# rofuyu/exp-trmf-nips16

Hardware: AMD Instinct MI355X
Metric: als_iterations_per_sec (higher is better)
Workload: dtype f32

## Files before the change

### exp-trmf-nips16_amd/csrc/session.hpp

```cpp
#pragma once

#include "session_xphase.hpp"

extern "C" char **environ;

namespace trmf {

struct TrmfSessionImpl : SessionXPhase {
    ~TrmfSessionImpl() {
        if (stream) (void)hipStreamSynchronize(stream);
        if (side) (void)hipStreamSynchronize(side);
        if (aux_theta) (void)hipStreamSynchronize(aux_theta);
        for (auto &e : events) {
            hipEvent_t all[] = {e.f0, e.fk0, e.fk1, e.f1, e.xg1, e.x1, e.lv1};
            for (hipEvent_t ev : all) if (ev) (void)hipEventDestroy(ev);
        }
        for (hipEvent_t ev : {gx0, gx1, gx2, fs0, fs1, fs2, ts0, ts1}) if (ev) (void)hipEventDestroy(ev);
        release_p2p();
        for (hipEvent_t ev : {ov_b, ov_c[0], ov_c[1], ov_c[2], ov_c[3], emu_ready, emu_end}) if (ev) (void)hipEventDestroy(ev);
        if (side) (void)hipStreamDestroy(side);
        for (hipEvent_t ev : {theta_fork, theta_done}) if (ev) (void)hipEventDestroy(ev);
        if (cg_note) (void)hipHostFree(cg_note);
        StreamCache::release(aux_theta);
        StreamCache::release(stream);
// ... 73 lines not shown
        for (double x : h) acc += x;
        *out = acc;
        return 0;
    }
    int device_sum_squares(const real *dv, size_t count, double *out) { return launch_sum_squares(dv, count) || finish_sum_squares(out) ? kFail : 0; }
    size_t footprint_estimate() const {
        const size_t sz = sizeof(real), NVb = (size_t)(T + 1) * KP * sz, NHb = (size_t)(n + 1) * KP * sz;
        size_t b = dense ? 2 * (size_t)T * n * sz + (full ? (size_t)kGemmChunks * std::max(T, n) * KP * sz : 0)
                         : 2 * (size_t)nnz * (4 + sz) + ((size_t)T + n + 2) * 4;
        b += NVb + NHb + (size_t)(T + n) * k * sz;
        b += 11 * NVb + 4 * NVb;
        if (!full) b += (size_t)T * k * k * sz;
        if (full) b += NHb;
        if (generic) b += (size_t)std::min(kGenBlocks, std::max(n, 1)) * k * k * sz;
        b += (size_t)kLogCap * sizeof(DeviceIterLog) + ((size_t)32 << 20);
        return b + b / 16;
    }
    int create(const PyMatrix *Y, const uint32_t *lags, uint32_t lag_size, const PyMatrix *Wm,
               const PyMatrix *Hm, const PyMatrix *LVm) {
        T = (int)Y->rows; n = (int)Y->cols; k = (int)Wm->cols; nnz = Y->nnz;
        KP = padded_rank(k); NT = KP / kTile; KMAX = ((k + 7) / 8) * 8;
        generic = k > kMaxRank;
        nlag = (int)lag_size; midx = nlag ? (int)lags[nlag - 1] : 0;
        comm = active_comm();
        if (StreamCache::acquire(&stream)) return kFail;
        FillStreamScope fill(stream);
        dense = Y->type != TRMF_SPARSE;
        DevicePool::current().reserve(footprint_estimate());

        const double tu0 = now_s();
        if (!dense) {
            host_row_ptr.assign(Y->row_ptr, Y->row_ptr + (size_t)T + 1);
            host_col_ptr.assign(Y->col_ptr, Y->col_ptr + (size_t)n + 1);
            if (upload_ptr32(Yc_ptr, Y->col_ptr, (size_t)n + 1)) return kFail;
            if (Yc_idx.upload(Y->row_idx, nnz)) return kFail;
            if (Yc_val.upload((const real *)Y->val, nnz)) return kFail;
            if (upload_ptr32(Yr_ptr, Y->row_ptr, (size_t)T + 1)) return kFail;
            if (Yr_idx.upload(Y->col_idx, nnz)) return kFail;
            if (Yr_val.upload((const real *)Y->val_t, nnz)) return kFail;
            if (launch_sum_squares(Yr_val.p, nnz)) return kFail;
            bytes_uploaded += 2.0 * (double)nnz * (4 + sizeof(real)) + 8.0 * ((double)T + n + 2);
        } else {
            const size_t N = (size_t)T * n;
            if (Yd_tn.alloc(N, false) || Yd_nt.alloc(N, false)) return kFail;
            if (Y->type == TRMF_DENSE_ROWMAJOR) {
                if (HostStager::current().h2d(Yd_tn.p, Y->val, N * sizeof(real), stream)) return kFail;
                launch_transpose(Yd_tn.p, T, n, Yd_nt.p);
            } else {
                if (HostStager::current().h2d(Yd_nt.p, Y->val, N * sizeof(real), stream)) return kFail;
                launch_transpose(Yd_nt.p, n, T, Yd_tn.p);
            }
            if (launch_sum_squares(Yd_tn.p, N)) return kFail;
            bytes_uploaded += (double)N * sizeof(real);
        }
        if (lag_set.upload(lags, nlag)) return kFail;
        {
            const std::vector<uint32_t> steps = ar_lag_steps(lags, nlag);
            nsteps = (int)steps.size();
            if (lag_steps.upload(steps.data(), steps.size())) return kFail;
        }
        if (upload_padded(W, raw_W, (const real *)Wm->val, T)) return kFail;
        if (upload_padded(H, raw_H, (const real *)Hm->val, n)) return kFail;
        if (theta.upload((const real *)LVm->val, (size_t)nlag * k)) return kFail;
        bytes_uploaded += ((double)T + n + nlag) * k * sizeof(real);
        t_upload_s = now_s() - tu0;

        if (xstate.alloc(1) || log.alloc(kLogCap)) return kFail;
        if (full && (Bf.alloc((size_t)n * KP) || GSf.alloc((size_t)k * k) || Uf.alloc((size_t)k * k) || GSx.alloc((size_t)k * k + kHvGramPad) ||
                     sgram_part.alloc((size_t)kSmallGramBlocks * k * k)))
            return kFail;
        if (comm->world > 1 && count_ranks_per_device()) return kFail;
        if (alloc_time_scratch()) return kFail;

        events.resize(kEventRing);
        for (auto &e : events) {
            hipEvent_t *all[] = {&e.f0, &e.fk0, &e.fk1, &e.f1, &e.xg1, &e.x1, &e.lv1};
            for (hipEvent_t *ev : all) { *ev = nullptr; TRMF_HIP_CHECK(hipEventCreate(ev)); }
        }
        for (hipEvent_t *ev : {&gx0, &gx1, &gx2, &fs0, &fs1, &fs2, &ts0, &ts1}) TRMF_HIP_CHECK(hipEventCreate(ev));
        if (gramx_times.alloc((size_t)8 * comm->world)) return kFail;
        if (comm->world == 1) { gramx_mode = kGramxShard; fs_mode = kShardOn; }
        if (const char *e = test_env("TRMF_GRAMX")) gramx_mode = (e[0] == 'r') ? kGramxReplicate : kGramxShard;
        if (const char *e = test_env("TRMF_FSHARD")) fs_mode = (e[0] == 'r') ? kShardOff : kShardOn;
        if (finish_sum_squares(&ysq_acc)) return kFail;
        set_trYTY();
        raw_W.release(); raw_H.release(); sumsq_part.release();
        if (comm->world > 1) {
            std::vector<uint64_t> off(comm->world + 1);
            for (int r = 0; r <= comm->world; r++) off[r] = (uint64_t)r * 2 * sizeof(double);
            if (comm->allgatherv(gramx_times.p, off.data(), stream)) return kFail;
            TRMF_HIP_CHECK(hipStreamSynchronize(stream));
        }
        if (nlag > 0 && theta_overlap_pays() && !test_env("TRMF_NO_OVERLAP")) (void)ensure_aux();
        created = true;
        return autotune();
    }

    int alloc_time_scratch() {
        const size_t NV = (size_t)T * KP;
        if (full && dense && gemm_part.alloc((size_t)kGemmChunks * (size_t)std::max(T, n) * KP)) return kFail;
        if (Bv.alloc(NV) || g.alloc(NV) || s.alloc(NV) || r.alloc(NV) ||
            d0.alloc(NV) || d1.alloc(NV) || Hd.alloc(NV) || r1.alloc(NV) || Hd1.alloc(NV) || w_new.alloc(NV) ||
            lossrow.alloc(T))
            return kFail;
        const int nchunk = std::max(1, (T - midx + kThetaChunk - 1) / kThetaChunk);
        const int npairs = nlag * (nlag + 1) / 2 + nlag;
        if (theta_part.alloc((size_t)k * nchunk * std::max(npairs, 1))) return kFail;
        if (nlag && allow_dyn_lds(theta_gram_kernel, theta_gram_lds(), "Theta Gram (max lag too large)")) return kFail;
        if (nlag && theta_solve_lds() > kLdsMax) {
            if (theta_scratch.alloc((size_t)k * ((size_t)nlag * nlag + nlag), false)) return kFail;
        } else if (nlag && allow_dyn_lds(theta_solve_kernel, theta_solve_lds(), "Theta solve (too many lags)")) return kFail;
        if (generic) {
            if (gen_scratch.alloc((size_t)std::min(kGenBlocks, std::max(n, 1)) * k * k, false)) return kFail;
            if (allow_dyn_lds(gram_generic_kernel<true>, gram_generic_lds(k), "generic F-solve") ||
                allow_dyn_lds(gram_generic_kernel<false>, gram_generic_lds(k), "generic Gram build")) return kFail;
        }

        nbe = (int)std::min<size_t>(kMaxPartials, (NV + 255) / 256);
        rpb = std::max(1, 256 / k);
        nba = std::min(kMaxPartials, (T + rpb - 1) / rpb);
        if (full && !generic) {
            const int blocks = ((T + kApplyTile - 1) / kApplyTile + 3) / 4, passes = (blocks + 511) / 512;
            nba = std::max(1, (blocks + passes - 1) / passes);
            const size_t need = apply_shared_lds_bytes(KP);
            int rc = 0;
            if (!with_nt(NT, [&](auto N) { rc = allow_dyn_lds(apply_shared_mfma_kernel<decltype(N)::value>, need, "shared-Gram product"); })) return unsupported_rank();
            if (rc) return kFail;
        }
        tile_TI = 0; nbt = 1; persist_state = 0; persist_shard_state = 0; persist_failed = false; persist_note.clear(); snap_iter = -1;
        {
            int TI = hv_tile_rows(k);
            tile_nth = 256;
            if (const char *e = test_env("TRMF_HV_TI")) TI = std::max(1, std::min(TI, atoi(e)));
            const bool fits32 = (uint64_t)(T + 1) * KP * sizeof(real) < 0x7fffffffull;
            const bool tiles_ok = !generic && fits32 && !test_env("TRMF_NO_HV_TILE");
            const char *tk = test_env("TRMF_TILE");
            if (tiles_ok && comm->world == 1 && !(tk && tk[0] == 'n') && !test_env("TRMF_HV_TI")) {
                hipDeviceProp_t prop;
                int dev = 0;
                TRMF_HIP_CHECK(hipGetDevice(&dev));
                TRMF_HIP_CHECK(hipGetDeviceProperties(&prop, dev));
                const int cus = std::max(1, prop.multiProcessorCount), rows_wide = hv_tile_rows(k, 512), need = (T + cus - 1) / cus;
                int wide_TI = 0;
                const int maxcg = (int)std::min<long long>(max_cg_iter, (long long)T * k);
                const char *pe = getenv("TRMF_PERSIST");
                const bool persist_wanted = !(pe && atoi(pe) == 0) && maxcg <= kCgHistCap;
                if (tk && tk[0] == 'w') wide_TI = std::min(rows_wide, std::max(need, TI + 1));
                else if (persist_wanted && (T + TI - 1) / TI > cus && need <= rows_wide &&
                         persist_lds_bytes(need, midx, KP, nlag, k, (T + need - 1) / need) <= kLdsMax) wide_TI = need;
                if (wide_TI > 0 && hv_tile_lds_bytes(wide_TI, midx, KP, nlag, k) <= 64 * 1024) { TI = wide_TI; tile_nth = 512; }
            }
            if (tiles_ok && hv_tile_lds_bytes(TI, midx, KP, nlag, k) <= (tile_nth == 512 ? 64 : 48) * 1024) {
                tile_TI = TI;
                nbt = (T + TI - 1) / TI;
            } else tile_nth = 256;
        }
        gpacked = !full && !generic && tile_TI == 0 && !test_env("TRMF_GRAM_FULL");
        const size_t gelems = gpacked ? packed_gram_elems(k) : (size_t)k * k;
        if (G.alloc((full ? 1 : (size_t)T * gelems) + kHvGramPad)) return kFail;
        if (gpacked) {
            const size_t need = (size_t)apply_stages(k) * 512 * sizeof(real);
            if (allow_dyn_lds(apply_kernel<true, 5>, need, "packed cached-Gram product") ||
                allow_dyn_lds(apply_kernel<true, 10>, need, "packed cached-Gram product") ||
                allow_dyn_lds(apply_kernel<true, 17>, need, "packed cached-Gram product"))
                return kFail;
        }
// ... 184 lines not shown
        TRMF_HIP_CHECK(hipDeviceSynchronize());
        return autotune();
    }
    bool decisions_pending() const {
        if (comm->world <= 1 || full) return false;
        if (fs_mode == kShardMeasure && period_H > 0) return true;
        if (period_W <= 0) return false;
        if (x_form < 0) return true;
        const bool rep_gram = tile_TI > 0 ? x_form == kXRep : (!uts && !cg_shard);
        return rep_gram && !cg_shard && gramx_mode == kGramxMeasure;
    }
    struct TunedDecisions {
        int fs_mode, gramx_mode, x_form, tuned_iters;
        float x_ms[kXForms]; double x_ms_all[kXForms];
        std::vector<int> x_cands;
        std::string persist_note;
    };
    static std::map<std::string, TunedDecisions> &decision_cache() { static std::map<std::string, TunedDecisions> c; return c; }
    static std::mutex &decision_mu() { static std::mutex m; return m; }
    std::string decision_key() const {
        std::string key = std::to_string(T) + "," + std::to_string(n) + "," + std::to_string(k) + "," + std::to_string(nnz) + "," + std::to_string(nlag) + "," +
                          std::to_string(midx) + "," + std::to_string(sizeof(real)) + "," + std::to_string(full) + std::to_string(dense) + "," + std::to_string(comm->id) + "," +
                          std::to_string(comm->world) + "," + std::to_string(period_W > 0) + std::to_string(period_H > 0);
        for (char **e = ::environ; e && *e; e++) if (!strncmp(*e, "TRMF_", 5)) { key += ";"; key += *e; }
        return key;
    }
    int autotune() {
        tuned_iters = 0; decisions_from_cache = false;
        if (const char *e = getenv("TRMF_AUTOTUNE")) if (atoi(e) == 0) return 0;
        if (!decisions_pending()) return 0;
        const std::string key = decision_key();
        {
            std::lock_guard<std::mutex> lk(decision_mu());
            auto it = decision_cache().find(key);
            if (it != decision_cache().end() && it->second.x_cands == x_cands) {
                const TunedDecisions &d = it->second;
                fs_mode = d.fs_mode; gramx_mode = d.gramx_mode; x_form = d.x_form; persist_note = d.persist_note;
                for (int f = 0; f < kXForms; f++) { x_ms[f] = d.x_ms[f]; x_ms_all[f] = d.x_ms_all[f]; }
                x_calls = 2 * (int)x_cands.size();
                decisions_from_cache = true;
                if (!decisions_pending()) {
                    if (verbose && comm->rank == 0) fprintf(stderr, ">> %s\n", describe().c_str());
                    return 0;
                }
                decisions_from_cache = false;
            }
        }
        DevBuf<real> W0, H0, T0;
        SyncStreamOnExit drain(stream);
        const size_t nw = (size_t)(T + 1) * KP, nh = (size_t)(n + 1) * KP, nt = (size_t)nlag * k;
        if (W0.alloc(nw, false) || H0.alloc(nh, false) || T0.alloc(nt, false)) return kFail;
        TRMF_HIP_CHECK(hipMemcpyAsync(W0.p, W.p, nw * sizeof(real), hipMemcpyDeviceToDevice, stream));
        TRMF_HIP_CHECK(hipMemcpyAsync(H0.p, H.p, nh * sizeof(real), hipMemcpyDeviceToDevice, stream));
        if (nt) TRMF_HIP_CHECK(hipMemcpyAsync(T0.p, theta.p, nt * sizeof(real), hipMemcpyDeviceToDevice, stream));
        const int v = verbose, it0 = iter;
        const bool ln = log_norms;
        verbose = 0; log_norms = false;
        int rc = 0;
        for (; tuned_iters < kAutotuneMax && decisions_pending() && rc == 0; tuned_iters++) rc = run(1);
        verbose = v; log_norms = ln; iter = it0;
        if (rc) return kFail;
        TRMF_HIP_CHECK(hipMemcpyAsync(W.p, W0.p, nw * sizeof(real), hipMemcpyDeviceToDevice, stream));
        TRMF_HIP_CHECK(hipMemcpyAsync(H.p, H0.p, nh * sizeof(real), hipMemcpyDeviceToDevice, stream));
        if (nt) TRMF_HIP_CHECK(hipMemcpyAsync(theta.p, T0.p, nt * sizeof(real), hipMemcpyDeviceToDevice, stream));
        TRMF_HIP_CHECK(hipStreamSynchronize(stream));
        if (sync()) return kFail;
        if (!decisions_pending()) {
            TunedDecisions d{fs_mode, gramx_mode, x_form, tuned_iters, {}, {}, x_cands, persist_note};
            for (int f = 0; f < kXForms; f++) { d.x_ms[f] = x_ms[f]; d.x_ms_all[f] = x_ms_all[f]; }
            std::lock_guard<std::mutex> lk(decision_mu());
            decision_cache()[key] = d;
        }
        if (verbose && comm->rank == 0) fprintf(stderr, ">> %s\n", describe().c_str());
        return 0;
    }
    std::string describe_split() const {
        if (!longF.any() && !longX.any()) return "";
        char t[224];
        snprintf(t, sizeof t, "; split rows: F %zu rows in %u items (>= %u entries), X %zu rows in %u items (>= %u entries)", longF.rows.size(), longF.nitems,
                 longF.thresh, longX.rows.size(), longX.nitems, longX.thresh);
        return t;
    }
    std::string describe_lag() const {
        if (!lag_lasso()) return "; lag penalty: ridge";
        char t[96];
        snprintf(t, sizeof t, "; lag penalty: lasso l1=%g refit=%d", lambdaLagL1, lag_refit);
        return t;
    }
    std::string describe() const { return describe_forms() + describe_split() + describe_lag(); }
    std::string describe_forms() const {
        char buf[640];
        if (comm->world <= 1) {
            snprintf(buf, sizeof buf, "1 rank; X-solve %s", generic ? "unfused; generic kernels for rank > 64 (Gram build, F-solve)"
                     : tile_TI <= 0 ? "unfused (AR tile + cached-Gram product per CG step)"
                     : persist_state == 1 ? "fused, one persistent kernel per solve" : persist_state == 0 ? "fused (not run yet)" : "fused, one launch per CG step");
            std::string d(buf);
            if (!generic && tile_TI > 0) { snprintf(buf, sizeof buf, "; %d tiles of %d timestamps, %d threads", nbt, tile_TI, tile_nth); d += buf; }
            return persist_note.empty() ? d : d + " (" + persist_note + ")";
        }
        const bool fused = tile_TI > 0;
        std::string x;
        if (full) x = "full-observation path (shared Gram)";
        else if (fused && ts_possible) x = std::string("fused CG ") + x_form_name(x_form) + (x_form == kXRep && persist_state == 1 ? " (one persistent kernel per solve on every rank)" : "");
        else if (fused) x = "fused CG replicated (too few tiles to shard over time)";
        else if (uts) x = std::string("unfused CG ") + x_form_name(x_form);
        else x = cg_shard ? "unfused CG, cached-Gram product sharded (H d rows gathered per step)" : "unfused CG replicated";
        std::string meas;
        for (int f : x_cands) {
            char t[96];
            snprintf(t, sizeof t, "%s%s %.3f ms", meas.empty() ? "" : ", ", x_form_name(f), x_ms_all[f]);
            meas += t;
        }
        const bool rep_gram = !full && (fused ? x_form == kXRep : (!uts && !cg_shard));
        snprintf(buf, sizeof buf, "%d ranks; F rows %s%s; X-side Gram rows %s; %s%s%s%s; peer-to-peer transport %s%s%s; decided %s%d set-up iterations",
                 comm->world, fs_mode == kShardOff ? "replicated" : fs_mode == kShardOn ? "sharded + all-gather of H" : "sharded (undecided)",
                 (fs_mode == kShardOn && fchunks >= 2) ? " in overlapped chunks" : "",
                 !rep_gram ? "own timestamps only (never gathered)" : gramx_mode == kGramxReplicate ? "replicated" : gramx_mode == kGramxShard ? "sharded + all-gather of G" : "sharded (undecided)",
                 x.c_str(), meas.empty() ? "" : " [slowest rank's X phase: ", meas.c_str(), meas.empty() ? "" : "]",
                 p2p.on ? "available" : "unavailable", p2p.note.empty() ? "" : ": ", p2p.note.c_str(),
                 decisions_from_cache ? "by an earlier session of this process (cached), " : "in ", tuned_iters);
        return persist_note.empty() ? std::string(buf) : std::string(buf) + " (" + persist_note + ")";
    }

    int run(int iters) {
        if (comm->world == 1 && snap_iter < 0 && period_W > 0 && iters > 0 && tile_TI > 0 && !persist_failed) {
            const int maxcg = (int)std::min<long long>(max_cg_iter, (long long)T * k);
            FillStreamScope fill(stream);
            if (maxcg <= kCgHistCap && persist_usable(maxcg) && take_snapshot()) return kFail;
        }
        for (int it = 0; it < iters; it++) {
            const int iter1 = ++iter;
            DeviceIterLog *L = log.p + ((iter1 - 1) % kLogCap);
            PhaseEvents &ev = events[(iter1 - 1) % kEventRing];
            ev_on = ev_period > 0 && (iter1 % ev_period) == 0;
            if (ev_valid.size() != (size_t)kEventRing) ev_valid.assign(kEventRing, 0);
            ev_valid[(iter1 - 1) % kEventRing] = ev_on ? 1 : 0;
            static const DeviceIterLog blank = [] { DeviceIterLog b; std::memset(&b, 0, sizeof b); b.normF = b.normX = b.normLV = -1; return b; }();
            const bool doF = period_H > 0 && (iter1 % period_H) == 0;
            const bool doX = period_W > 0 && (iter1 % period_W) == 0;
            const bool doL = period_Lag > 0 && (iter1 % period_Lag) == 0;
            const bool device_log = doX && !log_norms && !verbose;
            if (!device_log) TRMF_HIP_CHECK(hipMemcpyAsync(L, &blank, sizeof blank, hipMemcpyHostToDevice, stream));
            TRMF_EVREC(ev.f0, stream);
            if (doF) {
                if (full ? fsolve_full(ev) : fsolve(ev)) return kFail;
                if (log_norms || verbose) log_norm(H.p, (size_t)n * KP, &L->normF);
                if (verbose) fprintf(stderr, ">> iter %d F %g\n", iter1, host_double(&L->normF));
            } else {
                TRMF_EVREC(ev.fk0, stream);
                TRMF_EVREC(ev.fk1, stream);
            }
            TRMF_EVREC(ev.f1, stream);
            if (!doX) TRMF_EVREC(ev.xg1, stream);
            if (doX) {
                if (join_theta()) return kFail;
                xg1_event = ev_on ? ev.xg1 : nullptr;
                const int xrc = xsolve(device_log ? &L->x : nullptr, device_log ? &L->normF : nullptr);
                xg1_event = nullptr;
                if (xrc) return kFail;
                if (log_norms || verbose) log_norm(W.p, (size_t)T * KP, &L->normX);
                if (!device_log)
                    TRMF_HIP_CHECK(hipMemcpyAsync(&L->x, xstate.p, sizeof(XState), hipMemcpyDeviceToDevice, stream));
                if (verbose) {
                    fprintf(stderr, ">> iter %d X %g\n", iter1, host_double(&L->normX));
                    if (verbose >= 2) {
                        XState hx;
                        (void)hipMemcpy(&hx, xstate.p, sizeof hx, hipMemcpyDeviceToHost);
                        fprintf(stdout, "iter  1 act %5.3e pre %5.3e delta %5.3e f %5.3e |g| %5.3e CG %3d |g| %5.3e\n",
// ... 343 lines not shown
```

### exp-trmf-nips16_amd/csrc/session_state.hpp

```cpp
#pragma once

#include <algorithm>
#include <chrono>
#include <cmath>
#include <cstring>
#include <map>
#include <memory>
#include <mutex>
#include <type_traits>
#include <vector>

#include "../../include/trmf_abi.h"
#include "comm.hpp"
#include "dev_buf.hpp"
#include "full_kernels.hpp"
#include "generic_kernels.hpp"
#include "resident_kernels.hpp"
#include "theta_kernels.hpp"

namespace trmf {

std::shared_ptr<Comm> active_comm();

template <int... Vs, class F> bool dispatch_int(int v, F &&f) {
// ... 65 lines not shown
    hipEvent_t ts0 = nullptr, ts1 = nullptr;
    int ar_TI = 64, nbar = 1;
    DevBuf<real> arbase;
    XParams xp{};
    static bool test_knobs() { static const bool on = getenv("TRMF_TEST") != nullptr; return on; }
    static int unsupported_rank() { set_error("unsupported rank"); return kFail; }
    static const char *test_env(const char *name) {
        if (test_knobs()) return getenv(name);
        if (getenv(name)) {
            static std::mutex mu; static std::map<std::string, bool> told;
            std::lock_guard<std::mutex> lk(mu);
            if (!told[name]) { told[name] = true; fprintf(stderr, "[trmf] %s is a test knob: ignored unless TRMF_TEST is set\n", name); }
        }
        return nullptr;
    }

    double *pbase_override = nullptr;
    static constexpr int kSumsqBlocks = 1024;
    DevBuf<double> sumsq_part;

    std::vector<uint64_t> host_row_ptr, host_col_ptr;
    double ysq_acc = 0;

    double t_upload_s = 0;
    double bytes_uploaded = 0;
    DevBuf<real> raw_W, raw_H;
    static double now_s() { return std::chrono::duration<double>(std::chrono::steady_clock::now().time_since_epoch()).count(); }
    bool created = false;

    static double sum_squares(const real *v, uint64_t count) {
        double acc = 0;
        for (uint64_t e = 0; e < count; e++) acc += (double)v[e] * (double)v[e];
        return acc;
    }
    static double dense_rows_to_rowmajor(const PyMatrix *Y, std::vector<real> &tn) {
        const size_t R = Y->rows, C = Y->cols;
        const real *v = (const real *)Y->val;
        tn.resize(R * C);
        if (Y->type == TRMF_DENSE_ROWMAJOR) std::memcpy(tn.data(), v, R * C * sizeof(real));
        else
            for (size_t j = 0; j < R; j++)
                for (size_t i = 0; i < C; i++) tn[j * C + i] = v[i * R + j];
        return 0;
    }
    void launch_transpose(const real *src, int rows, int cols, real *dst) {
        if (rows > 0 && cols > 0)
            hipLaunchKernelGGL(transpose_kernel, dim3((cols + 31) / 32, (rows + 31) / 32), dim3(32, 8), 0, stream, src, rows, cols, dst);
    }
    void set_trYTY() { trYTY = (full || dense) ? (double)(real)ysq_acc : ysq_acc; xp.trYTY = trYTY; }

    DevBuf<real> Yraw;
    DevBuf<real> tr_a, tr_b;
    DevBuf<double> tr_part;
    bool has_transform = false;

    bool ho_set = false;
    uint64_t ho_m = 0, ho_chunk = kHoStep;
    int ho_nb = 1;
    DevBuf<uint32_t> ho_row, ho_col;
    DevBuf<real> ho_val, ho_pred;
    DevBuf<double> ho_part, ho_sums;

    DevBuf<double> fc_table[2];
    DevBuf<real> fc_prev[2];
    int fc_cur = 0;
    uint64_t fc_rows = 0;
    enum { kGramxMeasure = 0, kGramxShard = 1, kGramxReplicate = 2 };
    int gramx_mode = kGramxMeasure, gramx_calls = 0;
    hipEvent_t gx0 = nullptr, gx1 = nullptr, gx2 = nullptr;
    DevBuf<double> gramx_times;
    enum { kShardMeasure = 0, kShardOn = 1, kShardOff = 2 };
    int fs_mode = kShardMeasure, fs_calls = 0;
    hipEvent_t fs0 = nullptr, fs1 = nullptr, fs2 = nullptr;
    static constexpr uint64_t kOverlapBytes = 16ull << 20;
    static constexpr int kMaxChunks = 4;
    hipStream_t side = nullptr;
    hipEvent_t emu_ready = nullptr, emu_end = nullptr;
    hipEvent_t ov_b = nullptr, ov_c[kMaxChunks] = {nullptr, nullptr, nullptr, nullptr};
    std::vector<uint64_t> fcut;
    int fchunks = 0;
    hipStream_t aux_theta = nullptr;
    hipEvent_t theta_fork = nullptr, theta_done = nullptr;
    bool theta_pending = false;
    double lambdaLagL1 = 0;
    int lag_refit = 0;
    DevBuf<double> lasso_scratch;
    DevBuf<int> lag_rec;
    bool lag_rec_valid = false;
    bool lag_lasso() const { return lambdaLagL1 > 0 || lag_refit != 0; }
    bool theta_overlap_pays() const { return (double)k * (double)T * (double)nlag * (double)nlag >= (test_env("TRMF_OVERLAP_ALWAYS") ? 0.0 : 1e9); }
    bool overlap_ok() { return !verbose && !log_norms && !test_env("TRMF_NO_OVERLAP") && theta_overlap_pays() && ensure_aux() == 0; }
    int ensure_aux() {
        if (aux_theta) return 0;
        if (StreamCache::acquire(&aux_theta)) return kFail;
        for (hipEvent_t *e : {&theta_fork, &theta_done})
            if (!*e) TRMF_HIP_CHECK(hipEventCreateWithFlags(e, hipEventDisableTiming));
        return 0;
    }
    int join_theta() {
        if (!theta_pending) return 0;
        theta_pending = false;
        TRMF_HIP_CHECK(hipStreamWaitEvent(stream, theta_done, 0));
        return 0;
    }
    static constexpr int kCgLook = 2;
    unsigned int *cg_note = nullptr;
    unsigned int cg_seq = 0;
    bool cg_note_failed = false;
    int ensure_cg_note() {
        if (cg_note || cg_note_failed) return cg_note ? 0 : kFail;
        void *p = nullptr;
        if (hipHostMalloc(&p, 64, hipHostMallocMapped) != hipSuccess) { (void)hipGetLastError(); cg_note_failed = true; return kFail; }
        cg_note = (unsigned int *)p;
        *cg_note = 0;
        return 0;
    }
    DevBuf<unsigned long long> ll_rec, ll_vec;
    DevBuf<long long> persist_prof;
    uint32_t persist_epoch = 1;
    int persist_state = 0;
    template <int KQ, bool SHARD = false, int NTH = 256> int persist_prepare(size_t lds) {
        const void *fn = reinterpret_cast<const void *>(&cg_persist_kernel<KQ, SHARD, NTH>);
        if (lds > kLdsMax) return 0;
        if (lds > kLdsDefault && hipFuncSetAttribute(fn, hipFuncAttributeMaxDynamicSharedMemorySize, (int)lds) != hipSuccess) { (void)hipGetLastError(); return 0; }
        int per_cu = 0, dev = 0;
        hipDeviceProp_t prop;
        if (hipOccupancyMaxActiveBlocksPerMultiprocessor(&per_cu, fn, NTH, lds) != hipSuccess || hipGetDevice(&dev) != hipSuccess ||
            hipGetDeviceProperties(&prop, dev) != hipSuccess) { (void)hipGetLastError(); return 0; }
        return std::min(per_cu, NTH == 256 ? 4 : 1) * prop.multiProcessorCount;
    }
    template <int KQ, bool SHARD = false, int NTH = 256> int persist_launch(const PersistArgs &pa, size_t lds) {
        hipLaunchKernelGGL((cg_persist_kernel<KQ, SHARD, NTH>), dim3(SHARD ? tsh_rank.ntiles : nbt), dim3(NTH), lds, stream, xp, xstate.p, pa);
        TRMF_HIP_CHECK(hipGetLastError());
        return 0;
    }
    int max_ranks_per_device = 1;
    int persist_shard_state = 0;
    bool persist_failed = false;
    std::string persist_note;
    bool cg_shard = false;
    static constexpr int kShardSlots = 4096;
    int apply_slots = 1;
    bool uts = false;
    TileShard ush{};
    std::vector<uint64_t> ubounds;
    DevBuf<double> umsg;
    double *umsg_ptr = nullptr;
    unsigned u_exchanges = 0;
    int u_tile0 = 0, u_ntiles = 0, u_tpr = 0, wn_slots = 1;
    struct PartialRef { int slot, kind; };

    struct LongRows {
        uint32_t thresh = 0xffffffffu, chunk = 1024;
        std::vector<uint32_t> rows, first;
        DevBuf<uint32_t> d_rows, d_first, d_items;
        DevBuf<uint32_t> d_order;
        uint32_t nitems = 0;
        uint64_t nnz_long = 0;
        bool skewed = false;
        bool any() const { return !rows.empty(); }
        void clear() { thresh = 0xffffffffu; skewed = false; rows.clear(); first.clear(); nitems = 0; nnz_long = 0; d_rows.release(); d_first.release(); d_items.release(); d_order.release(); }
        void range(uint32_t rb, uint32_t re, uint32_t &lo, uint32_t &hi) const {
            lo = (uint32_t)(std::lower_bound(rows.begin(), rows.end(), rb) - rows.begin());
            hi = (uint32_t)(std::lower_bound(rows.begin(), rows.end(), re) - rows.begin());
        }
    } longF, longX;
// ... 66 lines not shown
```

### exp-trmf-nips16_amd/csrc/session_xphase.hpp

```cpp
#pragma once

#include "session_fphase.hpp"

namespace trmf {

struct SessionXPhase : SessionFPhase {
    int setup_tile_messages() {
        tsh = TileShard{};
        tsh.rank = 0; tsh.world = 1; tsh.tile0 = 0; tsh.ntiles = nbt; tsh.nbt = nbt; tsh.tpr = std::max(nbt, 1);
        tsh.row_b = 0; tsh.row_e = T; tsh.slot_dbl = (unsigned)nbt * kRecDoubles; tsh.edge_off_dbl = tsh.slot_dbl;
        tsh_rank = tsh;
        ts_possible = false;
        tbounds.assign(comm->world + 1, (uint64_t)T);
        tbounds[0] = 0;
        size_t doubles = (size_t)std::max(nbt, 1) * kRecDoubles;
        const int W_ = comm->world;
        if (tile_TI > 0 && W_ > 1 && !full) {
            const int tpr = (nbt + W_ - 1) / W_;
            const long long last_rows = (long long)T - (long long)(W_ - 1) * tpr * tile_TI;
            if ((long long)(W_ - 1) * tpr < nbt && (long long)tpr * tile_TI >= midx && last_rows >= std::max(midx, 1)) {
                ts_possible = true;
                const size_t edge_bytes = (size_t)2 * kEdgeVecs * midx * KP * sizeof(real);
                tsh_rank.rank = comm->rank; tsh_rank.world = W_; tsh_rank.tpr = tpr;
                tsh_rank.tile0 = comm->rank * tpr; tsh_rank.ntiles = std::min(nbt, (comm->rank + 1) * tpr) - tsh_rank.tile0;
// ... 455 lines not shown
                    TRMF_HIP_CHECK(hipStreamSynchronize(stream));
                    int err = 0;
                    TRMF_HIP_CHECK(hipMemcpy(&err, &xstate.p->p2p_error, sizeof(int), hipMemcpyDeviceToHost));
                    if (err) {
                        if (getenv("TRMF_P2P_VERBOSE")) {
                            XState hx;
                            TRMF_HIP_CHECK(hipMemcpy(&hx, xstate.p, sizeof hx, hipMemcpyDeviceToHost));
                            fprintf(stderr, "[persist trial] rank %d: error %d, exchange %lld, tile %lld, missing %lld (1 records, 2 halo rows) %lld (tiles %d..%d of %d)\n",
                                    comm->rank, err, hx.p2p_diag[0], hx.p2p_diag[1], hx.p2p_diag[2], hx.p2p_diag[3], tsh_rank.tile0, tsh_rank.tile0 + tsh_rank.ntiles, nbt);
                        }
                        TRMF_HIP_CHECK(hipMemset(&xstate.p->p2p_error, 0, sizeof(int)));
                        x_ms[kXTsPersist] = 1e9f; persist_failed = true;
                        persist_note = "the persistent kernel's trial timed out";
                    }
                }
            } else if (xsolve_fused(shard, maxcg, log_x, log_n)) return kFail;
            if (timed && form == kXTsPersist && persist_failed) { timed = false; TRMF_HIP_CHECK(hipEventRecord(ts1, stream)); }
            return end_timed();
        }
        real *dbuf[2] = {d0.p, d1.p}, *rbuf[2] = {r.p, r1.p}, *hbuf[2] = {Hd.p, Hd1.p};
        double *Pb = pbase();
        const int ndot = (cg_shard || uts) ? comm->world * apply_slots : nba;
        const size_t NV = (size_t)T * KP;
        const size_t own_b = uts ? (size_t)ush.row_b * KP : 0, own_e = uts ? (size_t)ush.row_e * KP : NV;
        const size_t halo_b = uts ? (size_t)std::max(0, ush.row_b - midx) * KP : 0, halo_e = uts ? (size_t)std::min(T, ush.row_e + midx) * KP : NV;
        const int nbw = uts ? wn_slots : nbe, npw = uts ? comm->world * wn_slots : nbe;
        ArVecs av{};
        av.v = W.p;
        if (hv(av, -1, 0, 1, g.p, 0)) return kFail;
        hipLaunchKernelGGL(cg_init_kernel, dim3(nbe), dim3(256), 0, stream, xp, st, Pb, nbar, ndot, g.p,
                           s.p, rbuf[0], dbuf[0], halo_b, halo_e);
        av = ArVecs{};
        av.v = dbuf[0]; av.r_in = rbuf[0];
        if (hv(av, 0, 0, 0, hbuf[0], 1)) return kFail;
        const bool follow_u = uts && !p2p_use;
        int upto = follow_u ? std::min(maxcg, std::max(1, cg_pred)) : maxcg;
        const bool follow_note = comm->world == 1 && maxcg > kCgLook + 1 && maxcg < 128 && !test_env("TRMF_NO_CG_FOLLOW") && ensure_cg_note() == 0;
        const unsigned int seq = follow_note ? (++cg_seq & 0xffffffu) : 0u;
        bool note_live = follow_note;
        for (int it = 1; it <= maxcg; it++) {
            av.v = dbuf[(it - 1) & 1]; av.r_in = rbuf[(it - 1) & 1]; av.hd_in = hbuf[(it - 1) & 1];
            av.s = s.p; av.d_out = dbuf[it & 1]; av.r_out = rbuf[it & 1];
            av.note = follow_note ? cg_note : nullptr; av.note_seq = seq;
            if (hv(av, it, it == maxcg ? 1 : 0, 0, hbuf[it & 1], 1)) return kFail;
            if (note_live && it < maxcg && it > kCgLook) {
                const unsigned int need = (unsigned int)(it - kCgLook);
                const double t_wait = now_s();
                bool stopped = false;
                for (unsigned int spins = 0;; spins++) {
                    const unsigned int v = __atomic_load_n(cg_note, __ATOMIC_ACQUIRE);
                    if ((v >> 8) == seq) {
                        if (v & 1u) { stopped = true; break; }
                        if (((v >> 1) & 0x7fu) >= need) break;
                    }
                    if ((spins & 1023u) == 1023u && now_s() - t_wait > 2.0) { note_live = false; break; }
                    __builtin_ia32_pause();
                }
                if (stopped) break;
            }
            if (!follow_u) continue;
            if (it == upto && it < maxcg) {
                int stop = kCgRunning;
                TRMF_HIP_CHECK(hipMemcpyAsync(&stop, &xstate.p->stop_it, sizeof(int), hipMemcpyDeviceToHost, stream));
                TRMF_HIP_CHECK(hipStreamSynchronize(stream));
                if (stop != kCgRunning) { cg_pred = stop; break; }
                upto = std::min(maxcg, upto + 2);
            } else if (it == maxcg) cg_pred = maxcg;
        }
        hipLaunchKernelGGL(wnew_kernel, dim3(nbw), dim3(256), 0, stream, xp, st, W.p, s.p, g.p, rbuf[0], rbuf[1], w_new.p, Pb, own_b, own_e,
                           uts ? comm->rank * wn_slots : 0);
        if (uts && uts_exchange(-1, cg_direct ? 1 : 0, cg_direct ? s.p : nullptr, nullptr, nullptr, {{P_GS, 2}, {P_SR, 2}, {P_SS, 2}})) return kFail;
        if (cg_direct) {
            av = ArVecs{};
            av.v = s.p;
            if (hv(av, -1, 0, 0, hbuf[0], 1)) return kFail;
        }
        hipLaunchKernelGGL(accept_kernel, dim3(nbw), dim3(256), 0, stream, xp, st, Pb, npw, ndot, (const double *)nullptr, w_new.p,
                           W.p, log_x, log_n, own_b, own_e, cg_direct ? 1 : 0);
        TRMF_HIP_CHECK(hipGetLastError());
        if (uts && gather_rows(W.p, ubounds, (size_t)KP * sizeof(real))) return kFail;
        return end_timed();
    }

    size_t theta_gram_lds() const { return theta_gram_lds_bytes(midx); }
    size_t theta_solve_lds() const { return (size_t)(nlag * nlag + nlag) * sizeof(real); }
    size_t theta_lasso_lds() const { return theta_lasso_doubles(nlag) * sizeof(double); }
    int ensure_lasso_buffers() {
        if (nlag == 0) return 0;
        FillStreamScope fill(stream);
        if (!lag_rec.p && lag_rec.alloc((size_t)k * kLagRec)) return kFail;
        if (theta_lasso_lds() > kLdsMax) {
            const size_t need = (size_t)k * theta_lasso_doubles(nlag);
            if (!lasso_scratch.p) DevicePool::current().reserve(need * sizeof(double));
            if (!lasso_scratch.p && lasso_scratch.alloc(need, false)) return kFail;
            return 0;
        }
        return allow_dyn_lds(theta_lasso_kernel<false>, theta_lasso_lds(), "lasso Theta solve");
    }
    int theta_solve(hipStream_t stream) {
        if (nlag == 0) return 0;
        const int nchunk = std::max(1, (T - midx + kThetaChunk - 1) / kThetaChunk);
        const int npairs = nlag * (nlag + 1) / 2 + nlag;
        const size_t lds1 = theta_gram_lds();
        hipLaunchKernelGGL(theta_gram_kernel, dim3(k, nchunk), dim3(256), lds1, stream, W.p, T, KP, lag_set.p,
                           nlag, midx, npairs, theta_part.p);
        if (lag_lasso()) {
            if (lasso_scratch.p)
                hipLaunchKernelGGL(theta_lasso_kernel<true>, dim3(k), dim3(256), 0, stream, theta_part.p, nchunk, nlag, npairs, lambdaLag,
                                   lambdaLagL1, lag_refit, theta.p, lasso_scratch.p, lag_rec.p);
            else
                hipLaunchKernelGGL(theta_lasso_kernel<false>, dim3(k), dim3(256), theta_lasso_lds(), stream, theta_part.p, nchunk, nlag, npairs,
                                   lambdaLag, lambdaLagL1, lag_refit, theta.p, (double *)nullptr, lag_rec.p);
            TRMF_HIP_CHECK(hipGetLastError());
            lag_rec_valid = true;
            return 0;
        }
        lag_rec_valid = false;
        const size_t lds2 = theta_scratch.p ? 0 : theta_solve_lds();
        hipLaunchKernelGGL(theta_solve_kernel, dim3(k), dim3(256), lds2, stream, theta_part.p, nchunk, nlag,
                           npairs, lambdaLag, theta.p, theta_scratch.p);
        TRMF_HIP_CHECK(hipGetLastError());
        return 0;
    }
};

}
```

### exp-trmf-nips16_amd/csrc/theta_kernels.hpp

```cpp
#pragma once

#include "common.hpp"

namespace trmf {

constexpr int kThetaChunk = 512;
constexpr int kMaxLags = 1024;

__device__ __forceinline__ void theta_decode_pair(int p, int nlag, int &a, int &b, bool &rhs) {
    if (p < nlag) { rhs = true; a = p; b = p; return; }
    rhs = false;
    int q = p - nlag, row = 0, len = nlag;
    while (q >= len) { q -= len; row++; len--; }
    a = row; b = row + q;
}

constexpr int kThetaTile = 4;
constexpr int kThetaRows = 4;
__host__ __device__ inline size_t theta_gram_lds_bytes(int midx) {
    return ((size_t)(kThetaChunk + midx + kThetaRows) * sizeof(real) + 15) / 16 * 16 + (size_t)256 * 16 * sizeof(double);
}
__global__ __launch_bounds__(256) void theta_gram_kernel(const real *__restrict__ W, int T, int KP,
                                                         const uint32_t *__restrict__ lag_set,
                                                         int nlag, int midx, int npairs,
                                                         double *__restrict__ part) {
    extern __shared__ __attribute__((aligned(16))) unsigned char smem_raw[];
    real *series = reinterpret_cast<real *>(smem_raw);
    double *red = reinterpret_cast<double *>(smem_raw + (((size_t)(kThetaChunk + midx + kThetaRows) * sizeof(real) + 15) / 16 * 16));
    const int t = blockIdx.x, ch = blockIdx.y, nchunk = gridDim.y;
    const int i0 = midx + ch * kThetaChunk;
    const int i1 = min(T, i0 + kThetaChunk);
    const int lo = i0 - midx;
    const int tp = colpos(t, KP / kTile);
    for (int i = lo + threadIdx.x; i < i1; i += 256) series[i - lo] = W[(size_t)i * KP + tp];
    __syncthreads();
    const int NA = (nlag + kThetaTile - 1) / kThetaTile;
    const int ntiles = NA * (NA + 1) / 2 + NA;
    const int S = max(1, 256 / ntiles);
    double *out = part + ((size_t)t * nchunk + ch) * npairs;
    for (int base = 0; base < ntiles; base += 256 / S) {
        const int tile = base + (int)threadIdx.x / S, slice = (int)threadIdx.x % S;
        const bool live = tile < ntiles && (int)threadIdx.x < (256 / S) * S;
        int ta = 0, tb = 0;
        bool rhs = false;
        if (live) {
            if (tile >= NA * (NA + 1) / 2) { rhs = true; tb = tile - NA * (NA + 1) / 2; }
            else { int q = tile, len = NA; while (q >= len) { q -= len; ta++; len--; } tb = ta + q; }
        }
        int la[kThetaTile], lb[kThetaTile];
#pragma unroll
        for (int u = 0; u < kThetaTile; u++) {
            la[u] = rhs ? 0 : (int)lag_set[min(kThetaTile * ta + u, nlag - 1)];
            lb[u] = (int)lag_set[min(kThetaTile * tb + u, nlag - 1)];
        }
        double acc[kThetaTile][kThetaTile];
#pragma unroll
        for (int u = 0; u < kThetaTile; u++)
#pragma unroll
            for (int v = 0; v < kThetaTile; v++) acc[u][v] = 0;
        bool runs = live;
#pragma unroll
        for (int u = 1; u < kThetaTile; u++)
            runs = runs && (rhs || la[u] == la[0] + u) && lb[u] == lb[0] + u;
        if (runs) {
            constexpr int R = kThetaRows, Wn = R + kThetaTile - 1;
            for (int i = i0 + slice * R; i < i1; i += S * R) {
                real wa[Wn], wb[Wn];
                const real *pa = series + (i - la[0] - (kThetaTile - 1) - lo), *pb = series + (i - lb[0] - (kThetaTile - 1) - lo);
#pragma unroll
                for (int m = 0; m < Wn; m++) { wb[m] = pb[m]; wa[m] = rhs ? series[i - lo + min(m, R - 1)] : pa[m]; }
#pragma unroll
                for (int r = 0; r < R; r++) {
                    if (i + r >= i1) break;
#pragma unroll
                    for (int u = 0; u < kThetaTile; u++) {
                        if (rhs && u > 0) break;
                        const real su = rhs ? wa[r] : wa[r - u + kThetaTile - 1];
#pragma unroll
                        for (int v = 0; v < kThetaTile; v++) {
                            const real prod = su * wb[r - v + kThetaTile - 1];
                            acc[u][v] += (double)prod;
                        }
                    }
                }
            }
        } else if (live) {
            const int nrow = rhs ? 1 : kThetaTile;
            for (int i = i0 + slice; i < i1; i += S) {
                real sa[kThetaTile], sb[kThetaTile];
#pragma unroll
                for (int u = 0; u < kThetaTile; u++) { sa[u] = series[i - la[u] - lo]; sb[u] = series[i - lb[u] - lo]; }
#pragma unroll
                for (int u = 0; u < kThetaTile; u++)
                    if (u < nrow) {
#pragma unroll
                        for (int v = 0; v < kThetaTile; v++) {
                            const real prod = sa[u] * sb[v];
                            acc[u][v] += (double)prod;
                        }
                    }
            }
        }
        __syncthreads();
#pragma unroll
        for (int u = 0; u < kThetaTile; u++)
#pragma unroll
            for (int v = 0; v < kThetaTile; v++) red[(size_t)threadIdx.x * 16 + u * kThetaTile + v] = acc[u][v];
        __syncthreads();
        if (live && slice == 0) {
#pragma unroll
            for (int u = 0; u < kThetaTile; u++)
#pragma unroll
                for (int v = 0; v < kThetaTile; v++) {
                    const int a = kThetaTile * ta + u, b = kThetaTile * tb + v;
                    if (b >= nlag || (!rhs && (a >= nlag || a > b)) || (rhs && u > 0)) continue;
                    double sum = 0;
                    for (int sl = 0; sl < S; sl++) sum += red[(size_t)(threadIdx.x + sl) * 16 + u * kThetaTile + v];
                    const int p = rhs ? b : nlag + a * nlag - a * (a - 1) / 2 + (b - a);
                    out[p] = sum;
                }
        }
    }
}

__device__ __forceinline__ double theta_sum_pair(const double *__restrict__ part, int nchunk, int npairs, int t, int p) {
    double acc = 0;
#pragma unroll 8
    for (int ch = 0; ch < nchunk; ch++) acc += part[((size_t)t * nchunk + ch) * npairs + p];
    return acc;
}

template <typename E, bool CHECK> __device__ __forceinline__ bool theta_chol_solve(E *A, E *y, int nlag, int lane) {
    for (int j = 0; j < nlag; j++) {
        if (CHECK) { const E piv = A[j * nlag + j]; if (!(piv > E(0)) || !isfinite(piv)) return false; }
        const E ajj = sqrt(A[j * nlag + j]);
        __syncthreads();
        for (int c = j + lane; c < nlag; c += 64) A[j * nlag + c] = (c == j) ? ajj : A[j * nlag + c] / ajj;
        __syncthreads();
        for (int c = j + 1 + lane; c < nlag; c += 64) {
            const E ujc = A[j * nlag + c];
            int s = j + 1;
            for (; s + 3 <= c; s += 4) {
                E u[4], a[4];
#pragma unroll
                for (int q = 0; q < 4; q++) { u[q] = A[j * nlag + s + q]; a[q] = A[(s + q) * nlag + c]; }
#pragma unroll
                for (int q = 0; q < 4; q++) A[(s + q) * nlag + c] = a[q] - u[q] * ujc;
            }
            for (; s <= c; s++) A[s * nlag + c] -= A[j * nlag + s] * ujc;
        }
        __syncthreads();
    }
    for (int q = 0; q < nlag; q++) {
        if (lane == 0) y[q] = y[q] / A[q * nlag + q];
        __syncthreads();
        for (int i = q + 1 + lane; i < nlag; i += 64) y[i] -= A[q * nlag + i] * y[q];
        __syncthreads();
    }
    for (int q = nlag - 1; q >= 0; q--) {
        if (lane == 0) y[q] = y[q] / A[q * nlag + q];
        __syncthreads();
        for (int i = lane; i < q; i += 64) y[i] -= A[i * nlag + q] * y[q];
        __syncthreads();
    }
    return true;
}

__global__ __launch_bounds__(256) void theta_solve_kernel(const double *__restrict__ part, int nchunk,
                                                         int nlag, int npairs, double lambdaLag,
                                                         real *__restrict__ theta, real *__restrict__ scratch) {
    extern __shared__ __attribute__((aligned(16))) unsigned char smem_raw[];
    real *A = scratch ? scratch + (size_t)blockIdx.x * ((size_t)nlag * nlag + nlag) : reinterpret_cast<real *>(smem_raw);
    real *y = A + nlag * nlag;
    const int t = blockIdx.x, lane = threadIdx.x;
    for (int p = threadIdx.x; p < npairs; p += 256) {
        const double acc = theta_sum_pair(part, nchunk, npairs, t, p);
        int a, b; bool rhs;
        theta_decode_pair(p, nlag, a, b, rhs);
        if (rhs) y[a] = (real)acc;
        else {
            real v = (real)acc;
            if (a == b) v = (real)((double)v + lambdaLag);
            A[a * nlag + b] = v;
            A[b * nlag + a] = v;
        }
    }
    __syncthreads();
    if (threadIdx.x >= 64) return;
    theta_chol_solve<real, false>(A, y, nlag, lane);
    for (int a = lane; a < nlag; a += 64) theta[(size_t)t * nlag + a] = y[a];
}

#if defined(TRMF_F32)
constexpr double kLassoEps = 1e-7;
#else
constexpr double kLassoEps = 1e-13;
#endif
constexpr int kLassoMaxSweeps = 1000;
constexpr int kLagRec = 4;
__host__ __device__ inline size_t theta_lasso_doubles(int nlag) { return (size_t)nlag * nlag + 3 * (size_t)nlag; }

__device__ __forceinline__ double lasso_soft(double rho, double l1) { return rho > l1 ? rho - l1 : rho < -l1 ? rho + l1 : 0.0; }

template <bool GLOB>
__global__ __launch_bounds__(256) void theta_lasso_kernel(const double *__restrict__ part, int nchunk, int nlag, int npairs,
                                                         double lambdaLag, double lambdaL1, int refit, real *__restrict__ theta,
                                                         double *__restrict__ scratch, int *__restrict__ rec) {
    extern __shared__ __attribute__((aligned(16))) unsigned char smem_raw[];
    constexpr bool glob = GLOB;
    double *G = GLOB ? scratch + (size_t)blockIdx.x * theta_lasso_doubles(nlag) : reinterpret_cast<double *>(smem_raw);
    double *b = G + (size_t)nlag * nlag, *r = b + nlag, *th = r + nlag;
    const int t = blockIdx.x, lane = threadIdx.x;
    for (int p = threadIdx.x; p < npairs; p += 256) {
        const double acc = theta_sum_pair(part, nchunk, npairs, t, p);
        int a, c; bool rhs;
        theta_decode_pair(p, nlag, a, c, rhs);
        if (rhs) b[a] = acc;
        else { G[a * nlag + c] = acc; G[c * nlag + a] = acc; }
    }
    for (int i = threadIdx.x; i < nlag; i += 256) {
        const double v = (double)theta[(size_t)t * nlag + i];
        th[i] = isfinite(v) ? v : 0.0;
    }
    __syncthreads();
    for (int i = threadIdx.x; i < nlag; i += 256) {
        double acc = b[i];
        for (int j = 0; j < nlag; j++) acc -= G[j * nlag + i] * th[j];
        r[i] = acc;
    }
    __syncthreads();
    if (threadIdx.x >= 64) return;
    int sweeps = 0, capped = 0;
    for (;;) {
        double dmax = 0, tmax = 0;
        for (int j = 0; j < nlag; j++) {
            const double gjj = G[j * nlag + j], thj = th[j], den = gjj + lambdaLag;
            double tn = (den > 0 && isfinite(den)) ? lasso_soft(r[j] + gjj * thj, lambdaL1) / den : 0.0;
            if (!isfinite(tn)) tn = 0.0;
            const double delta = tn - thj;
            if (delta != 0) {
                if (glob) __syncthreads();
                for (int i = lane; i < nlag; i += 64) r[i] -= delta * G[j * nlag + i];
                if (lane == 0) th[j] = tn;
                if (glob) __syncthreads();
            }
            dmax = fmax(dmax, fabs(delta)); tmax = fmax(tmax, fabs(tn));
        }
        sweeps++;
        if (dmax <= kLassoEps * fmax(1.0, tmax)) break;
        if (sweeps >= kLassoMaxSweeps) { capped = 1; break; }
    }
    int *idx = reinterpret_cast<int *>(r);
    int m = 0;
    __syncthreads();
    for (int base = 0; base < nlag; base += 64) {
        const bool on = base + lane < nlag && (real)th[base + lane] != real(0);
        const unsigned long long mask = __ballot(on);
        if (on) idx[m + __popcll(mask & ((1ull << lane) - 1ull))] = base + lane;
        m += __popcll(mask);
    }
    __syncthreads();
    int skipped = 0;
    if (refit && m > 0) {
        for (int base = 0; base < m * m; base += 64) {
            const int o = base + lane, p = o / m, q = o - p * m;
            double v = 0;
            if (o < m * m) v = G[idx[p] * nlag + idx[q]] + (p == q ? lambdaLag : 0.0);
            __syncthreads();
            if (o < m * m) G[o] = v;
            __syncthreads();
        }
        for (int base = 0; base < m; base += 64) {
            const int p = base + lane;
            double v = 0;
            if (p < m) v = b[idx[p]];
// ... 29 lines not shown
```

Baseline: 1215.

## Solve small ridge Theta systems in registers and restructure Theta Gram reduction

Adds a register-resident Cholesky solve for the ridge lag system when nlag is at most 32, with one lane per column and cross-lane reads via readlane, in place of the LDS-based solve that synchronises after every step. The Theta Gram kernel now caches lag indices in LDS, decodes tiles in closed form, unrolls the series load, and runs the slice reduction in parallel across all threads using a padded transposed layout. The solves also switch to explicit fma. The intent is to cut barrier and LDS traffic in the Theta phase. It adds template instantiations and register pressure, and because of fma rounding the results may differ slightly.

```diff
diff --git a/exp-trmf-nips16_amd/csrc/session.hpp b/exp-trmf-nips16_amd/csrc/session.hpp
--- a/exp-trmf-nips16_amd/csrc/session.hpp
+++ b/exp-trmf-nips16_amd/csrc/session.hpp
@@ -179,6 +179,7 @@
         if (comm->world == 1) { gramx_mode = kGramxShard; fs_mode = kShardOn; }
         if (const char *e = test_env("TRMF_GRAMX")) gramx_mode = (e[0] == 'r') ? kGramxReplicate : kGramxShard;
         if (const char *e = test_env("TRMF_FSHARD")) fs_mode = (e[0] == 'r') ? kShardOff : kShardOn;
+        if (const char *e = test_env("TRMF_THETA_SOLVE")) theta_force_lds = std::string(e) == "lds";
         if (finish_sum_squares(&ysq_acc)) return kFail;
         set_trYTY();
         raw_W.release(); raw_H.release(); sumsq_part.release();
@@ -529,8 +530,13 @@
         return t;
     }
     std::string describe_lag() const {
-        if (!lag_lasso()) return "; lag penalty: ridge";
         char t[96];
+        if (!lag_lasso()) {
+            if (nlag == 0) return "; lag penalty: ridge";
+            if (const int cls = theta_reg_class()) snprintf(t, sizeof t, "; lag penalty: ridge (solve in registers, class %d)", cls);
+            else snprintf(t, sizeof t, "; lag penalty: ridge (solve in %s)", theta_scratch.p ? "global scratch" : "LDS");
+            return t;
+        }
         snprintf(t, sizeof t, "; lag penalty: lasso l1=%g refit=%d", lambdaLagL1, lag_refit);
         return t;
     }
diff --git a/exp-trmf-nips16_amd/csrc/session_state.hpp b/exp-trmf-nips16_amd/csrc/session_state.hpp
--- a/exp-trmf-nips16_amd/csrc/session_state.hpp
+++ b/exp-trmf-nips16_amd/csrc/session_state.hpp
@@ -171,6 +171,7 @@
     hipStream_t aux_theta = nullptr;
     hipEvent_t theta_fork = nullptr, theta_done = nullptr;
     bool theta_pending = false;
+    bool theta_force_lds = false;
     double lambdaLagL1 = 0;
     int lag_refit = 0;
     DevBuf<double> lasso_scratch;
diff --git a/exp-trmf-nips16_amd/csrc/session_xphase.hpp b/exp-trmf-nips16_amd/csrc/session_xphase.hpp
--- a/exp-trmf-nips16_amd/csrc/session_xphase.hpp
+++ b/exp-trmf-nips16_amd/csrc/session_xphase.hpp
@@ -561,7 +561,7 @@
         return end_timed();
     }
 
-    size_t theta_gram_lds() const { return theta_gram_lds_bytes(midx); }
+    size_t theta_gram_lds() const { return theta_gram_lds_bytes(midx, nlag); }
     size_t theta_solve_lds() const { return (size_t)(nlag * nlag + nlag) * sizeof(real); }
     size_t theta_lasso_lds() const { return theta_lasso_doubles(nlag) * sizeof(double); }
     int ensure_lasso_buffers() {
@@ -575,6 +575,10 @@
             return 0;
         }
         return allow_dyn_lds(theta_lasso_kernel<false>, theta_lasso_lds(), "lasso Theta solve");
+    }
+    int theta_reg_class() const {
+        if (nlag == 0 || nlag > kThetaRegMax || theta_force_lds) return 0;
+        return nlag <= 8 ? 8 : nlag <= 16 ? 16 : 32;
     }
     int theta_solve(hipStream_t stream) {
         if (nlag == 0) return 0;
@@ -595,6 +599,14 @@
             return 0;
         }
         lag_rec_valid = false;
+        if (const int cls = theta_reg_class()) {
+            auto go = [&](auto kern) { hipLaunchKernelGGL(kern, dim3(k), dim3(256), 0, stream, theta_part.p, nchunk, nlag, npairs, lambdaLag, theta.p); };
+            if (cls == 8) go(theta_solve_reg_kernel<8>);
+            else if (cls == 16) go(theta_solve_reg_kernel<16>);
+            else go(theta_solve_reg_kernel<32>);
+            TRMF_HIP_CHECK(hipGetLastError());
+            return 0;
+        }
         const size_t lds2 = theta_scratch.p ? 0 : theta_solve_lds();
         hipLaunchKernelGGL(theta_solve_kernel, dim3(k), dim3(256), lds2, stream, theta_part.p, nchunk, nlag,
                            npairs, lambdaLag, theta.p, theta_scratch.p);
diff --git a/exp-trmf-nips16_amd/csrc/theta_kernels.hpp b/exp-trmf-nips16_amd/csrc/theta_kernels.hpp
--- a/exp-trmf-nips16_amd/csrc/theta_kernels.hpp
+++ b/exp-trmf-nips16_amd/csrc/theta_kernels.hpp
@@ -17,8 +17,19 @@
 
 constexpr int kThetaTile = 4;
 constexpr int kThetaRows = 4;
-__host__ __device__ inline size_t theta_gram_lds_bytes(int midx) {
-    return ((size_t)(kThetaChunk + midx + kThetaRows) * sizeof(real) + 15) / 16 * 16 + (size_t)256 * 16 * sizeof(double);
+constexpr int kThetaRedStride = 257;
+__host__ __device__ inline size_t theta_gram_series_bytes(int midx) {
+    return ((size_t)(kThetaChunk + midx + kThetaRows) * sizeof(real) + 15) / 16 * 16;
+}
+__host__ __device__ inline size_t theta_gram_lds_bytes(int midx, int nlag) {
+    return theta_gram_series_bytes(midx) + (size_t)16 * kThetaRedStride * sizeof(double) + (size_t)(256 + nlag) * sizeof(int);
+}
+__device__ __forceinline__ void theta_decode_tile(int q, int NA, int &ta, int &tb) {
+    const float h = (float)(2 * NA + 1);
+    int r = min(NA - 1, max(0, (int)((h - sqrtf(h * h - 8.0f * (float)q)) * 0.5f)));
+    while (r > 0 && r * NA - r * (r - 1) / 2 > q) r--;
+    while ((r + 1) * NA - (r + 1) * r / 2 <= q) r++;
+    ta = r; tb = r + (q - (r * NA - r * (r - 1) / 2));
 }
 __global__ __launch_bounds__(256) void theta_gram_kernel(const real *__restrict__ W, int T, int KP,
                                                          const uint32_t *__restrict__ lag_set,
@@ -26,16 +37,26 @@
                                                          double *__restrict__ part) {
     extern __shared__ __attribute__((aligned(16))) unsigned char smem_raw[];
     real *series = reinterpret_cast<real *>(smem_raw);
-    double *red = reinterpret_cast<double *>(smem_raw + (((size_t)(kThetaChunk + midx + kThetaRows) * sizeof(real) + 15) / 16 * 16));
+    double *red = reinterpret_cast<double *>(smem_raw + theta_gram_series_bytes(midx));
+    int *blocks = reinterpret_cast<int *>(red + 16 * kThetaRedStride);
+    int *lags = blocks + 256;
     const int t = blockIdx.x, ch = blockIdx.y, nchunk = gridDim.y;
     const int i0 = midx + ch * kThetaChunk;
     const int i1 = min(T, i0 + kThetaChunk);
     const int lo = i0 - midx;
     const int tp = colpos(t, KP / kTile);
-    for (int i = lo + threadIdx.x; i < i1; i += 256) series[i - lo] = W[(size_t)i * KP + tp];
+    for (int i = threadIdx.x; i < nlag; i += 256) lags[i] = (int)lag_set[i];
+    for (int i = lo + threadIdx.x; i < i1; i += 4 * 256) {
+        real w[4];
+#pragma unroll
+        for (int u = 0; u < 4; u++) w[u] = i + u * 256 < i1 ? W[(size_t)(i + u * 256) * KP + tp] : real(0);
+#pragma unroll
+        for (int u = 0; u < 4; u++) if (i + u * 256 < i1) series[i + u * 256 - lo] = w[u];
+    }
     __syncthreads();
     const int NA = (nlag + kThetaTile - 1) / kThetaTile;
-    const int ntiles = NA * (NA + 1) / 2 + NA;
+    const int ntri = NA * (NA + 1) / 2;
+    const int ntiles = ntri + NA;
     const int S = max(1, 256 / ntiles);
     double *out = part + ((size_t)t * nchunk + ch) * npairs;
     for (int base = 0; base < ntiles; base += 256 / S) {
@@ -44,14 +65,14 @@
         int ta = 0, tb = 0;
         bool rhs = false;
         if (live) {
-            if (tile >= NA * (NA + 1) / 2) { rhs = true; tb = tile - NA * (NA + 1) / 2; }
-            else { int q = tile, len = NA; while (q >= len) { q -= len; ta++; len--; } tb = ta + q; }
+            if (tile >= ntri) { rhs = true; tb = tile - ntri; }
+            else theta_decode_tile(tile, NA, ta, tb);
         }
         int la[kThetaTile], lb[kThetaTile];
 #pragma unroll
         for (int u = 0; u < kThetaTile; u++) {
-            la[u] = rhs ? 0 : (int)lag_set[min(kThetaTile * ta + u, nlag - 1)];
-            lb[u] = (int)lag_set[min(kThetaTile * tb + u, nlag - 1)];
+            la[u] = rhs ? 0 : lags[min(kThetaTile * ta + u, nlag - 1)];
+            lb[u] = lags[min(kThetaTile * tb + u, nlag - 1)];
         }
         double acc[kThetaTile][kThetaTile];
 #pragma unroll
@@ -105,20 +126,22 @@
 #pragma unroll
         for (int u = 0; u < kThetaTile; u++)
 #pragma unroll
-            for (int v = 0; v < kThetaTile; v++) red[(size_t)threadIdx.x * 16 + u * kThetaTile + v] = acc[u][v];
-        __syncthreads();
-        if (live && slice == 0) {
-#pragma unroll
-            for (int u = 0; u < kThetaTile; u++)
-#pragma unroll
-                for (int v = 0; v < kThetaTile; v++) {
-                    const int a = kThetaTile * ta + u, b = kThetaTile * tb + v;
-                    if (b >= nlag || (!rhs && (a >= nlag || a > b)) || (rhs && u > 0)) continue;
-                    double sum = 0;
-                    for (int sl = 0; sl < S; sl++) sum += red[(size_t)(threadIdx.x + sl) * 16 + u * kThetaTile + v];
-                    const int p = rhs ? b : nlag + a * nlag - a * (a - 1) / 2 + (b - a);
-                    out[p] = sum;
-                }
+            for (int v = 0; v < kThetaTile; v++) red[(u * kThetaTile + v) * kThetaRedStride + (int)threadIdx.x] = acc[u][v];
+        if (live && slice == 0) blocks[tile - base] = ta | (tb << 16);
+        __syncthreads();
+        for (int o = threadIdx.x; o < (256 / S) * 16; o += 256) {
+            const int tl = o >> 4, e = o & 15, rt = base + tl;
+            if (rt >= ntiles) break;
+            const int u = e / kThetaTile, v = e % kThetaTile;
+            const bool rr = rt >= ntri;
+            const int ra = blocks[tl] & 0xffff, rb = blocks[tl] >> 16;
+            const int a = kThetaTile * ra + u, b = kThetaTile * rb + v;
+            if (b >= nlag || (!rr && (a >= nlag || a > b)) || (rr && u > 0)) continue;
+            const double *src = red + e * kThetaRedStride + tl * S;
+            double sum = 0;
+            for (int sl = 0; sl < S; sl++) sum += src[sl];
+            const int p = rr ? b : nlag + a * nlag - a * (a - 1) / 2 + (b - a);
+            out[p] = sum;
         }
     }
 }
@@ -130,6 +153,8 @@
     return acc;
 }
 
+template <typename E> __device__ __forceinline__ E theta_nmsub(E a, E u, E c) { return fma(-u, c, a); }
+
 template <typename E, bool CHECK> __device__ __forceinline__ bool theta_chol_solve(E *A, E *y, int nlag, int lane) {
     for (int j = 0; j < nlag; j++) {
         if (CHECK) { const E piv = A[j * nlag + j]; if (!(piv > E(0)) || !isfinite(piv)) return false; }
@@ -145,22 +170,22 @@
 #pragma unroll
                 for (int q = 0; q < 4; q++) { u[q] = A[j * nlag + s + q]; a[q] = A[(s + q) * nlag + c]; }
 #pragma unroll
-                for (int q = 0; q < 4; q++) A[(s + q) * nlag + c] = a[q] - u[q] * ujc;
+                for (int q = 0; q < 4; q++) A[(s + q) * nlag + c] = theta_nmsub(a[q], u[q], ujc);
             }
-            for (; s <= c; s++) A[s * nlag + c] -= A[j * nlag + s] * ujc;
+            for (; s <= c; s++) A[s * nlag + c] = theta_nmsub(A[s * nlag + c], A[j * nlag + s], ujc);
         }
         __syncthreads();
     }
     for (int q = 0; q < nlag; q++) {
         if (lane == 0) y[q] = y[q] / A[q * nlag + q];
         __syncthreads();
-        for (int i = q + 1 + lane; i < nlag; i += 64) y[i] -= A[q * nlag + i] * y[q];
+        for (int i = q + 1 + lane; i < nlag; i += 64) y[i] = theta_nmsub(y[i], A[q * nlag + i], y[q]);
         __syncthreads();
     }
     for (int q = nlag - 1; q >= 0; q--) {
         if (lane == 0) y[q] = y[q] / A[q * nlag + q];
         __syncthreads();
-        for (int i = lane; i < q; i += 64) y[i] -= A[i * nlag + q] * y[q];
+        for (int i = lane; i < q; i += 64) y[i] = theta_nmsub(y[i], A[i * nlag + q], y[q]);
         __syncthreads();
     }
     return true;
@@ -191,6 +216,79 @@
     for (int a = lane; a < nlag; a += 64) theta[(size_t)t * nlag + a] = y[a];
 }
 
+constexpr int kThetaRegMax = 32;
+__device__ __forceinline__ float theta_lane(float v, int l) { return __int_as_float(__builtin_amdgcn_readlane(__float_as_int(v), l)); }
+__device__ __forceinline__ double theta_lane(double v, int l) {
+    return __hiloint2double(__builtin_amdgcn_readlane(__double2hiint(v), l), __builtin_amdgcn_readlane(__double2loint(v), l));
+}
+template <typename E, int N> __device__ __forceinline__ E theta_chol_solve_reg(E (&col)[N], E yv, int nlag, int lane) {
+#pragma unroll
+    for (int j = 0; j < N; j++)
+        if (j < nlag) {
+            const E ajj = sqrt(theta_lane(col[j], j));
+            col[j] = lane == j ? ajj : col[j] / ajj;
+            const E ujc = col[j];
+#pragma unroll
+            for (int s = j + 1; s < N; s++) col[s] = theta_nmsub(col[s], theta_lane(ujc, s), ujc);
+        }
+#pragma unroll
+    for (int q = 0; q < N; q++)
+        if (q < nlag) {
+            const E zq = theta_lane(yv, q) / theta_lane(col[q], q);
+            yv = lane == q ? zq : lane > q ? theta_nmsub(yv, col[q], zq) : yv;
+        }
+    E x[N];
+#pragma unroll
+    for (int i = 0; i < N; i++) x[i] = theta_lane(yv, i);
+#pragma unroll
+    for (int q = N - 1; q >= 0; q--)
+        if (q < nlag) {
+            x[q] = x[q] / theta_lane(col[q], q);
+#pragma unroll
+            for (int i = 0; i < q; i++) x[i] = theta_nmsub(x[i], theta_lane(col[i], q), x[q]);
+        }
+    E out = E(0);
+#pragma unroll
+    for (int i = 0; i < N; i++) out = lane == i ? x[i] : out;
+    return out;
+}
+
+__device__ __forceinline__ double theta_sum_pair_wide(const double *__restrict__ part, int nchunk, int npairs, int t, int p) {
+    double acc = 0;
+    for (int c0 = 0; c0 < nchunk; c0 += 32) {
+        double v[32];
+#pragma unroll
+        for (int u = 0; u < 32; u++) v[u] = c0 + u < nchunk ? part[((size_t)t * nchunk + c0 + u) * npairs + p] : 0.0;
+#pragma unroll
+        for (int u = 0; u < 32; u++) if (c0 + u < nchunk) acc += v[u];
+    }
+    return acc;
+}
+
+template <int N>
+__global__ __launch_bounds__(256) void theta_solve_reg_kernel(const double *__restrict__ part, int nchunk, int nlag, int npairs,
+                                                             double lambdaLag, real *__restrict__ theta) {
+    __shared__ real sm[N * (N + 1) / 2 + N];
+    const int t = blockIdx.x, lane = threadIdx.x;
+    for (int p = threadIdx.x; p < npairs; p += 256) sm[p] = (real)theta_sum_pair_wide(part, nchunk, npairs, t, p);
+    __syncthreads();
+    if (threadIdx.x >= 64) return;
+    real col[N];
+#pragma unroll
+    for (int s = 0; s < N; s++) {
+        real v = real(0);
+        if (s < nlag && lane < nlag) {
+            const int a = min(s, lane), b = max(s, lane);
+            v = sm[nlag + a * nlag - a * (a - 1) / 2 + (b - a)];
+            if (s == lane) v = (real)((double)v + lambdaLag);
+        }
+        col[s] = v;
+    }
+    const real yv = lane < nlag ? sm[lane] : real(0);
+    const real x = theta_chol_solve_reg<real, N>(col, yv, nlag, lane);
+    if (lane < nlag) theta[(size_t)t * nlag + lane] = x;
+}
+
 #if defined(TRMF_F32)
 constexpr double kLassoEps = 1e-7;
 #else
```

New measurement: 1232, median of 6. +1.4%, better.
